# YiKwanwoo2/mycelium-fea-project

Hardware: AMD Instinct MI355X
Metric: DOF solved/sec + CG iters to 1e-8; SpMV achieved HBM GB/s vs roofline (higher is better)
Workload: dtype f64 (CG; f32 AMG V-cycle); 1 GPU; C3_1M: 6x8 tiles, 1062000 DOF, 1008054 free DOF, 364342 elements, load step 20/40; n_dof=1062000, n_free_dof=1008054, n_elems=364342, precond=gamg, parallelism=1gpu, cg_kernel=lanes, n_lanes=353600

## Files before the change

### mycelium-fea-project_amd/csrc/amg.hip

```cpp
#include "amg_dev.hpp"

namespace mfea {

__device__ __forceinline__ int64_t setup_block(int x1, int64_t nmain = -1) {
  if (!x1) return nmain < 0 ? xcd_block() : xcd_block_n(nmain);
  return (blockIdx.x & 7) ? -1 : (int64_t)(blockIdx.x >> 3);
}


template <int ND>
__device__ __forceinline__ double dinv_row(const AmgLevD& L, int64_t i) {
  const AmgMatD& A = L.A;
  double g = 0.0;
  if (i - (threadIdx.x & 63) < A.rg.hi) {
    int64_t base;
    int w;
    slice_of(A, i, base, w);
    if (i >= A.rg.lo && i < A.rg.hi) {
      double D[ND * ND], Di[ND * ND];
      bload<ND>(A.val32, A.npos, base, D);
      binv<ND>(D, Di);
#pragma unroll
      for (int c = 0; c < ND * ND; ++c) L.dinv32[i * (ND * ND) + c] = (float)Di[c];
      double rs[ND];
// ... 1265 lines not shown
      acc[2] = fma(r[a], r[a], acc[2]);
      acc[3] = fma(u[a], u[a], acc[3]);
    }
  }
  store_block_partial<BS>(acc, part_buf(part, FIRST ? 0 : ((j & 1) ^ 1)));
  if (FIRST && blockIdx.x == 0 && threadIdx.x == 0) {
    Slot s0;
    s0.v[0] = s0.v[1] = s0.v[2] = s0.v[3] = 0.0;
    s0.alpha = s0.beta = s0.res = 0.0;
    s0.flag = kInit;
    s0.pad = 0;
    slots[0] = s0;
  }
}

template <int ND, int BS>
__global__ __launch_bounds__(BS) void k_amg_rnorm(AmgCg cg, double* cpart) {
  double acc[4] = {0.0, 0.0, 0.0, 0.0};
  const int64_t stride = (int64_t)gridDim.x * BS;
  const int lane = threadIdx.x & 63;
  for (int64_t i = cg.lo64() + xcd_block() * BS + threadIdx.x; i - lane < cg.hi; i += stride) {
    if (i < cg.lo || i >= cg.hi) continue;
    double r[ND];
    vload<ND>(cg.r, i, r);
#pragma unroll
    for (int a = 0; a < ND; ++a) acc[2] = fma(r[a], r[a], acc[2]);
  }
  store_block_partial<BS>(acc, cpart);
}

template <int PU>
__global__ __launch_bounds__(64) void k_amg_gsum(const double* __restrict__ p, double* all, int rank, int zero_w,
                                                 double* gsend) {
  double S[4];
  wave_partials<PU>(p, S);
  const int lane = threadIdx.x;
  if (lane < zero_w && lane != rank) {
#pragma unroll
    for (int c = 0; c < 4; ++c) all[4 * lane + c] = 0.0;
// ... 4 lines not shown
      all[4 * rank + c] = S[c];
      gsend[c] = S[c];
    }
  }
}

template <int ND>
__global__ __launch_bounds__(kBlock) void k_amg_pack_u(AmgCg cg, AmgDist d) {
  const int64_t k = (int64_t)blockIdx.x * kBlock + threadIdx.x;
  if (k >= d.n_send) return;
  const int64_t i = d.send_rows[k];
#pragma unroll
  for (int a = 0; a < ND; ++a) d.usend[ND * k + a] = i >= 0 ? cg.u[ND * i + a] : 0.0;
}

template <int ND, int PU, int BS, bool DIST>
__global__ __launch_bounds__(BS) void k_amg_cg_update(int j, AmgLevD L0, AmgCg cg, Slot* slots,
                                                      SolveState* st, double* part, AmgDist d) {
  const int f0 = __builtin_nontemporal_load(&slots[j].flag);
  const double g0 = slots[j].v[0], a0 = slots[j].alpha;
  double tol2 = st->tol2;
  const int base_it = st->base, max_it = st->max_it, norm = st->norm;
  double S[4];
  if constexpr (DIST) {
    const int lane = threadIdx.x & 63;
    const double* g = d.gall[j & 1];
#pragma unroll
    for (int c = 0; c < 4; ++c) S[c] = wave_allsum(g[lane * 4 + c]);
  } else {
    wave_partials<PU>(part_buf(part, j & 1), S);
  }
  const int64_t stride = (int64_t)gridDim.x * BS;
  const int64_t i0 = cg.lo + (int64_t)blockIdx.x * BS + threadIdx.x;
  const bool x0_here = !cg.sweep && !L0.coarsest;
  const float om0 = x0_here ? (float)amg_omega_s(L0.omega) : 0.0f;
  double u[ND], w[ND], p[ND], s[ND], x[ND], r[ND];
  float Di[ND * ND];
  if (cg.hi > cg.lo) {
    const int64_t k = i0 < cg.hi ? i0 : cg.hi - 1;
    vload<ND>(cg.u, k, u);
    vload<ND>(cg.w, k, w);
    vload<ND>(cg.p, k, p);
    vload<ND>(cg.s, k, s);
    vload<ND>(cg.x, k, x);
    vload<ND>(cg.r, k, r);
    if (x0_here) dinv_load<ND>(L0.dinv32, k, Di);
  }
  if (norm == 1 && f0 == kInit) {
    tol2 = fmax(st->rtol2 * S[3], st->atol2);
    if (blockIdx.x == 0 && threadIdx.x == 0) {
      st->tol2 = tol2;
      st->res0 = S[3];
    }
  }
  const CgScalars cs = cg_scalars(S, f0, g0, a0, tol2, base_it + j, max_it, norm);
  cg_record(slots, j, S, cs);
  if (cs.status != kRun) return;
  const double alpha = cs.alpha, beta = cs.beta;
  for (int64_t i = i0; i < cg.hi; i += stride) {
    if (i != i0) {
      vload<ND>(cg.u, i, u);
      vload<ND>(cg.w, i, w);
      vload<ND>(cg.p, i, p);
      vload<ND>(cg.s, i, s);
      vload<ND>(cg.x, i, x);
      vload<ND>(cg.r, i, r);
      if (x0_here) dinv_load<ND>(L0.dinv32, i, Di);
    }
#pragma unroll
    for (int a = 0; a < ND; ++a) {
      p[a] = fma(beta, p[a], u[a]);
      s[a] = fma(beta, s[a], w[a]);
      x[a] = fma(alpha, p[a], x[a]);
      r[a] = fma(-alpha, s[a], r[a]);
    }
    vstore<ND>(cg.p, i, p);
    vstore<ND>(cg.s, i, s);
    vstore<ND>(cg.x, i, x);
    vstore<ND>(cg.r, i, r);
    if (x0_here) {
      float rf[ND], x0[ND];
#pragma unroll
      for (int a = 0; a < ND; ++a) rf[a] = (float)r[a];
      dinv_mul<ND>(Di, om0, rf, x0);
      vstore<ND>(L0.x, i, x0);
    } else {
      vcycle_entry<ND>(L0, cg, i, r);
    }
  }
}

template <int ND>
__global__ __launch_bounds__(kBlock) void k_amg_finish(AmgCg cg, double* __restrict__ x_row) {
// ... 444 lines not shown
    case 512: w_bs<ND, 512>(s, j, first, L0, cg, slots, part, d); break;
    case 576: w_bs<ND, 576>(s, j, first, L0, cg, slots, part, d); break;
    case 640: w_bs<ND, 640>(s, j, first, L0, cg, slots, part, d); break;
    case 704: w_bs<ND, 704>(s, j, first, L0, cg, slots, part, d); break;
    case 768: w_bs<ND, 768>(s, j, first, L0, cg, slots, part, d); break;
    case 1024: w_bs<ND, 1024>(s, j, first, L0, cg, slots, part, d); break;
    default: w_bs<ND, kCgBS>(s, j, first, L0, cg, slots, part, d); break;
  }
}
void launch_amg_cg_w(hipStream_t s, int nd, int j, bool first, const AmgLevD& L0, const AmgCg& cg,
                     Slot* slots, double* part, const AmgDist* d) {
  if (nd == 2) w_nd<2>(s, j, first, L0, cg, slots, part, d);
  else w_nd<3>(s, j, first, L0, cg, slots, part, d);
}

template <int ND>
static void rnorm_nd(hipStream_t s, const AmgCg& cg, double* cpart) {
  const dim3 g((unsigned)amg_w_grid(cg));
  switch (amg_w_block(cg)) {
    case 512: hipLaunchKernelGGL((k_amg_rnorm<ND, 512>), g, dim3(512), 0, s, cg, cpart); break;
    case 576: hipLaunchKernelGGL((k_amg_rnorm<ND, 576>), g, dim3(576), 0, s, cg, cpart); break;
    case 640: hipLaunchKernelGGL((k_amg_rnorm<ND, 640>), g, dim3(640), 0, s, cg, cpart); break;
    case 704: hipLaunchKernelGGL((k_amg_rnorm<ND, 704>), g, dim3(704), 0, s, cg, cpart); break;
    case 768: hipLaunchKernelGGL((k_amg_rnorm<ND, 768>), g, dim3(768), 0, s, cg, cpart); break;
    case 1024: hipLaunchKernelGGL((k_amg_rnorm<ND, 1024>), g, dim3(1024), 0, s, cg, cpart); break;
    default: hipLaunchKernelGGL((k_amg_rnorm<ND, kCgBS>), g, dim3(kCgBS), 0, s, cg, cpart); break;
  }
}
void launch_amg_rnorm(hipStream_t s, int nd, const AmgCg& cg, double* cpart) {
  if (nd == 2) rnorm_nd<2>(s, cg, cpart);
  else rnorm_nd<3>(s, cg, cpart);
}

void launch_amg_gsum(hipStream_t s, const AmgCg& cg, const double* part_q, const AmgDist& d, int q) {
  double* all = d.gall[q];
  const int r = d.rank, zw = d.zero_w;
  switch (pu_of_grid(amg_w_grid(cg))) {
    case 1: hipLaunchKernelGGL(k_amg_gsum<1>, dim3(1), dim3(64), 0, s, part_q, all, r, zw, d.gsend); break;
    case 2: hipLaunchKernelGGL(k_amg_gsum<2>, dim3(1), dim3(64), 0, s, part_q, all, r, zw, d.gsend); break;
    case 4: hipLaunchKernelGGL(k_amg_gsum<4>, dim3(1), dim3(64), 0, s, part_q, all, r, zw, d.gsend); break;
    default: hipLaunchKernelGGL(k_amg_gsum<8>, dim3(1), dim3(64), 0, s, part_q, all, r, zw, d.gsend); break;
  }
}

void launch_amg_pack_u(hipStream_t s, int nd, const AmgCg& cg, const AmgDist& d) {
  if (d.n_send <= 0) return;
  if (nd == 2) hipLaunchKernelGGL(k_amg_pack_u<2>, rows_grid(d.n_send), dim3(kBlock), 0, s, cg, d);
  else hipLaunchKernelGGL(k_amg_pack_u<3>, rows_grid(d.n_send), dim3(kBlock), 0, s, cg, d);
}

template <int ND, int BS, bool DIST>
static void upd_bs(hipStream_t s, int j, const AmgLevD& L0, const AmgCg& cg, Slot* slots,
                   SolveState* st, double* part, const AmgDist& d) {
  const int64_t gw = amg_w_grid(cg);
  int64_t gu = (cg.hi - cg.lo + BS - 1) / BS;
  gu = gu < 1 ? 1 : (gu > kCgMaxG ? kCgMaxG : gu);
  const dim3 g((unsigned)gu);
  switch (DIST ? 1 : pu_of_grid(gw)) {
    case 1: hipLaunchKernelGGL((k_amg_cg_update<ND, 1, BS, DIST>), g, dim3(BS), 0, s, j, L0, cg, slots, st, part, d); break;
    case 2: hipLaunchKernelGGL((k_amg_cg_update<ND, 2, BS, DIST>), g, dim3(BS), 0, s, j, L0, cg, slots, st, part, d); break;
    case 4: hipLaunchKernelGGL((k_amg_cg_update<ND, 4, BS, DIST>), g, dim3(BS), 0, s, j, L0, cg, slots, st, part, d); break;
    default: hipLaunchKernelGGL((k_amg_cg_update<ND, 8, BS, DIST>), g, dim3(BS), 0, s, j, L0, cg, slots, st, part, d); break;
  }
}
template <int ND>
static void upd_nd(hipStream_t s, int j, const AmgLevD& L0, const AmgCg& cg, Slot* slots,
                   SolveState* st, double* part, const AmgDist* d) {
  if (d) upd_bs<ND, kCgBS, true>(s, j, L0, cg, slots, st, part, *d);
  else upd_bs<ND, kCgBS, false>(s, j, L0, cg, slots, st, part, AmgDist{});
}
void launch_amg_cg_update(hipStream_t s, int nd, int j, const AmgLevD& L0, const AmgCg& cg, Slot* slots,
                          SolveState* st, double* part, const AmgDist* d) {
  if (nd == 2) upd_nd<2>(s, j, L0, cg, slots, st, part, d);
  else upd_nd<3>(s, j, L0, cg, slots, st, part, d);
}

void launch_amg_finish(hipStream_t s, int nd, const AmgCg& cg, double* x_row) {
  if (cg.hi <= cg.lo) return;
  if (nd == 2) hipLaunchKernelGGL(k_amg_finish<2>, rows_grid(cg.hi - cg.lo), dim3(kBlock), 0, s, cg, x_row);
  else hipLaunchKernelGGL(k_amg_finish<3>, rows_grid(cg.hi - cg.lo), dim3(kBlock), 0, s, cg, x_row);
}

template <class T>
__global__ __launch_bounds__(kBlock) void k_xpack(const T* __restrict__ src, const int32_t* __restrict__ idx,
                                                  int64_t n, int width, T* __restrict__ buf) {
  const int64_t k = (int64_t)blockIdx.x * kBlock + threadIdx.x;
  if (k >= n * width) return;
  const int64_t it = k / width, c = k - it * width;
  buf[k] = src[(int64_t)idx[it] * width + c];
// ... 92 lines not shown
```

### mycelium-fea-project_amd/csrc/amg_kernels.hpp

```cpp
#pragma once
#include <hip/hip_runtime.h>
#include <stdint.h>

#include "kernels.hpp"

namespace mfea {

struct RowRange {
  int64_t lo = 0, hi = 0;
  int64_t p0 = 0, p1 = 0;
  int64_t pf = 0, pl = 0;
  int64_t s0 = 0, s1 = 0;
  int64_t rows() const { return hi > lo ? hi - lo : 0; }
  __host__ __device__ int64_t lo64() const { return lo & ~(int64_t)63; }
  int64_t span() const { return hi > lo ? hi - lo64() : 0; }
  int64_t npos() const { return p1 > p0 ? p1 - p0 : 0; }
};

struct AmgMatD {
  int64_t n = 0;
  int64_t npos = 0;
  int32_t wmax = 0;
  RowRange rg;
  const int32_t* sptr = nullptr;
// ... 186 lines not shown
int amg_restrict_lanes(const AmgLevD& L);
int amg_op_lanes(const AmgLevD& L);
int amg_down_lanes(const AmgLevD& L);
int amg_up_lanes(const AmgLevD& L);
bool amg_compact_ok(const AmgLevD* lev, int nlev, int l0);
int amg_tail_level(const int64_t* rows, int nlev, int64_t max_rows);
void launch_amg_cg_init(hipStream_t s, int nd, const AmgLevD& L0, const AmgCg& cg, const double* b_row);
void launch_amg_cg_w(hipStream_t s, int nd, int j, bool first, const AmgLevD& L0, const AmgCg& cg,
                     Slot* slots, double* part, const AmgDist* d = nullptr);
void launch_amg_row0_inverse(hipStream_t s, const AmgCg& cg, int32_t* inv, int64_t n_rows);
void launch_amg_start(hipStream_t s, int nd, const SellOp& op, const uint8_t* code, double dy_top, double dy_bot,
                      const CgVecs& v, double* partials, unsigned* ticket, double* red_out, const AmgLevD& L0,
                      const AmgCg& cg, const int32_t* inv, double rtol, double atol, int norm, int max_it,
                      double reg, SolveState* st, double* zero, int64_t nzero);
void launch_amg_rnorm(hipStream_t s, int nd, const AmgCg& cg, double* cpart);
void launch_amg_gsum(hipStream_t s, const AmgCg& cg, const double* part_q, const AmgDist& d, int q);
void launch_amg_pack_u(hipStream_t s, int nd, const AmgCg& cg, const AmgDist& d);
void launch_amg_cg_update(hipStream_t s, int nd, int j, const AmgLevD& L0, const AmgCg& cg,
                          Slot* slots, SolveState* st, double* part,
                          const AmgDist* d = nullptr);
void launch_amg_finish(hipStream_t s, int nd, const AmgCg& cg, double* x_row);
int64_t amg_w_grid(const AmgCg& cg);

}
```

### mycelium-fea-project_amd/csrc/capi.hip

```cpp
#include <hip/hip_runtime.h>
#include <rccl/rccl.h>

#include <algorithm>
#include <deque>
#include <chrono>
#include <cmath>
#include <cstdio>
#include <cstring>
#include <memory>
#include <string>
#include <thread>
#include <vector>

#include "amg.hpp"
#include "amg_kernels.hpp"
#include "kernels.hpp"
#include "mfea_debug.h"
#include "mfea.h"
#include "partition.hpp"
#include "records.hpp"
#include "run.hpp"
#include "symbolic.hpp"

using namespace mfea;
// ... 128 lines not shown
  double amg_build_s = 0.0;
  double amg_excess_s = 0.0;
  bool amg_stale = false;
  bool amg_reused = false;
  int64_t amg_seen_gen = -1;
  DevBuf<int32_t> amg_i;
  DevBuf<double> amg_d;
  DevBuf<float> amg_f;
  std::vector<AmgLevD> amg_lev;
  DevBuf<AmgLevD> amg_levd;
  bool amg_om_own = false;
  bool amg_om_spatial = false;
  int amg_tail = 0;
  int amg_first = 1;
  AmgCg amg_cg;
  int amg_kind = MFEA_PC_GAMG;
  SweepPlan sweep;
  SweepD swd;
  DevBuf<int32_t> sw_i;
  DevBuf<float> sw_f;
  DevBuf<double> sw_y;
  const int32_t* amg_a0_ptr = nullptr;
  const int32_t* amg_a0_a = nullptr;
  AmgHalo amg_halo;
  AmgDist amg_dist;
  DevBuf<int32_t> amg_hi;
  DevBuf<double> amg_hd;
  AmgRank amg_rank;
  PosList g_a0;
  std::vector<int32_t> g_row0;
// ... 67 lines not shown
  int64_t op_gen = 0;
  struct {
    bool ok = false;
    int64_t act_gen = -1;
    Material mat{};
    int asm_kernel = -1;
  } k_from;
  int last_precond = -1;
  int64_t op_kept_steps = 0;
  int64_t amg_setup_kept = 0;
  int opt_amg_close = 1;
  int64_t amg_close_hits = 0;
  int amg_last_cycles = 0;
  int opt_amg_start = 1;
  int64_t amg_start_fused = 0;
  bool setup_skipped = false;
  Material graph_batch_mat{};
  bool asm_pending = false;
  DevBuf<double> d_dy;
  bool spec_on = false;
  bool spec_used = false;
  bool spec_launched = false;
  double spec_strain = 0.0;
  bool ev_on = false;
  double ev_strain = 0.0, ev_tie = 0.0, ev_lam_max = 0.0;
  int32_t ev_index = 0;
  int opt_event_scratch = 1;
  hipEvent_t poll[2] = {};
  int64_t n_active = 0;
  bool act_all = false;
// ... 1131 lines not shown
    const int64_t nf = nlev ? pl.lev[0].A.n : 0;
    pt.amg_cg.n = nf;
    pt.amg_cg.lo = rk && nlev ? rk->lo[0] : 0;
    pt.amg_cg.hi = rk && nlev ? rk->hi[0] : nf;
    pt.amg_cg.w_block = h->opt_amg_w_block;
    pt.amg_cg.w_k = amg_w_k(pl);
    pt.amg_cg.cycle = h->opt_amg_cycle;
    pt.amg_cg.coll = pt.amg_coll.kc;
    pt.amg_cg.row0 = I(row0 ? *row0 : pl.row0);
    pt.amg_cg.x = D((size_t)nd * nf);
    pt.amg_cg.p = D((size_t)nd * nf);
    pt.amg_cg.s = D((size_t)nd * nf);
    pt.amg_cg.w = D((size_t)nd * nf);
    pt.amg_cg.r = D((size_t)nd * nf);
    pt.amg_cg.u = F((size_t)nd * nf);
    pt.amg_mg = AmgMergeD{};
    if (pt.amg_mplan.on) {
      const AmgMerge& M = pt.amg_mplan;
      AmgMergeD& g = pt.amg_mg;
      g.n1 = M.n1;
      g.n2 = M.n2;
      g.DQ = mat(M.DQ, false, true);
      g.DQ.rg = row_range(M.DQ, 0, M.DQ.n);
      g.U = mat(M.U, false, true);
      g.U.rg = row_range(M.U, 0, M.U.n);
      g.dq_dst = I(M.dq_dst);
      g.dq_split = M.dq_split;
      g.dq_ext = I(M.dq_ext);
      g.dq_ptr = I(M.dq_l.ptr);
      g.dq_a = I(M.dq_l.a);
// ... 136 lines not shown
  w.up_pos = put(sp.up_pos);
  float* fp = pt.sw_f.ptr;
  w.pv = fp;
  w.dt = fp + (size_t)ne * nb2;
  w.lov = w.dt + (size_t)ne * ns;
  w.upv = w.lov + nlo * nb2;
  HIPC(hipMemsetAsync(fp, 0, pt.sw_f.n * sizeof(float), s));
  w.y = pt.sw_y.ptr;
  HIPC(hipMemsetAsync(w.y, 0, pt.sw_y.n * sizeof(double), s));
  pt.amg_cg.sweep = 1;
  HIPC(hipGetLastError());
  HIPC(hipStreamSynchronize(s));
  return 0;
}

void launch_precond(mfea_handle* h, Part& pt, const int32_t* gate) {
  if (pt.amg_cg.sweep) launch_sweep(h->stream, pt.amg.nd, pt.swd, pt.amg_cg, gate);
  else launch_amg_vcycle(h->stream, pt.amg.nd, pt.amg_lev.data(), (int)pt.amg_lev.size(), pt.amg_cg, pt.amg_tail, gate,
                         0, pt.amg_mg.on ? &pt.amg_mg : nullptr);
}

int upload_sweep(mfea_handle* h, Part& pt, int kind);

static bool active_subset(const std::vector<uint8_t>& a, const std::vector<uint8_t>& b) {
  if (a.size() != b.size()) return false;
  for (size_t e = 0; e < a.size(); ++e)
    if (a[e] && !b[e]) return false;
  return true;
}

std::string build_sweep_bounded(const AmgPlan& plan, int piece_len, SweepPlan& sp) {
  for (int m = piece_len;; m = std::max(1, m / 2)) {
    const std::string err = build_sweep(plan, m, sp);
    if (!err.empty() || sp.colors <= kSweepMaxColors) return err;
    if (m == 1) return "sweep plan: more than 32 colours";
// ... 70 lines not shown
  pt.amg_reused = false;
  if (!dm && pt.amg_lev.size() > 1) RC(enqueue_fmask(h, pt));
  clk.lap("floating mask");
  if (!dm) pt.amg_seen_gen = h->act_gen;
  pt.amg_sub_gen = dm ? -1 : h->act_sub_gen;
  pt.amg_key_count = (int64_t)std::count(key.begin(), key.end(), (uint8_t)1);
  ++pt.amg_gen;
  *rebuilt = true;
  return 0;
}

void enqueue_amg_iteration(mfea_handle* h, Part& pt, int j, bool profile) {
  hipStream_t s = h->stream;
  const int nd = pt.amg.nd;
  const AmgLevD& L0 = pt.amg_lev[0];
  launch_amg_cg_update(s, nd, j, L0, pt.amg_cg, pt.slots.ptr, pt.state.ptr, pt.cg_part.ptr);
  (void)profile;
  launch_precond(h, pt, nullptr);
  launch_amg_cg_w(s, nd, j, profile, L0, pt.amg_cg, pt.slots.ptr, pt.cg_part.ptr);
}

int xchg_u(mfea_handle* h) {
  hipStream_t s = h->stream;
  const int64_t nd = part0(h).amg.nd;
  if (h->world > 1) {
    Part& pt = part0(h);
    const PartPlan& pl = pt.plan;
    if (pl.xpeers.empty()) return 0;
    NCCLC(ncclGroupStart());
    for (size_t i = 0; i < pl.xpeers.size(); ++i) {
      if (pl.xsend_cnt[i])
        NCCLC(ncclSend(pt.amg_dist.usend + nd * pl.xsend_off[i], (size_t)(nd * pl.xsend_cnt[i]), ncclFloat64,
                       pl.xpeers[i], h->comm, s));
      if (pl.xrecv_cnt[i])
// ... 70 lines not shown
  HIPC(hipGetLastError());
  return xchg_sums(h, q);
}

int enqueue_amg_dist_chunk(mfea_handle* h, int chunk) {
  for (int j = 0; j < chunk; ++j) RC(enqueue_amg_dist_iteration(h, j));
  for (auto& pp : h->parts) launch_cg_advance(h->stream, chunk, pp->slots.ptr, pp->state.ptr, pp->mirror);
  HIPC(hipGetLastError());
  return 0;
}

void enqueue_amg_chunk(mfea_handle* h, Part& pt, int chunk, bool close) {
  hipStream_t s = h->stream;
  const int nd = pt.amg.nd;
  const AmgLevD& L0 = pt.amg_lev[0];
  for (int j = 0; j < chunk; ++j) {
    launch_precond(h, pt, nullptr);
    launch_amg_cg_w(s, nd, j, false, L0, pt.amg_cg, pt.slots.ptr, pt.cg_part.ptr);
    launch_amg_cg_update(s, nd, j + 1, L0, pt.amg_cg, pt.slots.ptr, pt.state.ptr, pt.cg_part.ptr);
  }
  if (close) launch_amg_rnorm(s, nd, pt.amg_cg, cg_part_buf(pt, 2));
  launch_cg_advance(s, chunk, pt.slots.ptr, pt.state.ptr, pt.mirror, 1, close ? cg_part_buf(pt, 2) : nullptr,
                    close ? (int)amg_w_grid(pt.amg_cg) : 0);
}

void enqueue_amg_setup(mfea_handle* h, Part& pt, double reg) {
  hipStream_t s = h->stream;
  const int nd = pt.amg.nd, nlev = (int)pt.amg_lev.size();
  const bool compact = pt.amg_cg.cycle == 1 && nlev > 1 && pt.amg_lev[0].compact;
  const bool fused = compact && h->opt_amg_fuse_setup && !pt.amg_cg.sweep;
  launch_amg_a0(s, nd, pt.amg_lev[0], sell_op(pt), pt.amg_cg.row0, pt.amg_a0_ptr, pt.amg_a0_a, reg,
                fused && pt.amg_lev[0].a0full);
  if (pt.amg_cg.sweep) {
    launch_sweep_setup(s, nd, pt.swd, pt.amg_lev[0]);
    return;
  }
// ... 8 lines not shown
  if (pt.amg_mg.on && !merged_done) launch_amg_merge_setup(s, nd, pt.amg_lev.data(), pt.amg_mg);
}

uint64_t fnv1a(uint64_t k, const void* p, size_t n) {
  const unsigned char* b = static_cast<const unsigned char*>(p);
  size_t i = 0;
  for (; i + 8 <= n; i += 8) {
    uint64_t w;
    std::memcpy(&w, b + i, 8);
    k = (k ^ w) * 1099511628211ULL;
  }
  for (; i < n; ++i) k = (k ^ b[i]) * 1099511628211ULL;
  return k;
}

void launch_precond(mfea_handle* h, Part& pt, const int32_t* gate);
int enqueue_post_work(mfea_handle* h, double max_strain);

void enqueue_amg_entry(mfea_handle* h, Part& pt, bool skip_init = false) {
  hipStream_t s = h->stream;
  const int nd = pt.amg.nd;
  const AmgLevD& L0 = pt.amg_lev[0];
  if (!skip_init) launch_amg_cg_init(s, nd, L0, pt.amg_cg, cg_vecs(pt).r[0]);
  launch_precond(h, pt, nullptr);
  launch_amg_cg_w(s, nd, 0, true, L0, pt.amg_cg, pt.slots.ptr, pt.cg_part.ptr);
  launch_amg_cg_update(s, nd, 0, L0, pt.amg_cg, pt.slots.ptr, pt.state.ptr, pt.cg_part.ptr);
}

void enqueue_step_head(mfea_handle* h, Part& pt, const mfea_solve_opts* o) {
  hipStream_t s = h->stream;
  const Pattern& P = pt.P;
  (void)hipMemcpyAsync(h->d_dy.ptr, h->h_red + 14, 2 * sizeof(double), hipMemcpyHostToDevice, s);
  AsmRhs q{};
  q.code = pt.code.ptr;
  q.top_end = P.n_free + P.n_top;
  q.bot_end = P.n_nodes - P.n_ghost;
  q.dyp = h->d_dy.ptr;
  q.nf = P.n_free;
  q.r = pt.r.ptr;
  q.x = pt.x.ptr;
  q.partials = pt.partials.ptr;
// ... 24 lines not shown
                           const mfea_solve_opts* head = nullptr, const mfea_solve_opts* start = nullptr,
                           int tail = -1, int tag = 0, bool close = false, bool skip_init = false) {
  hipStream_t s = h->stream;
  uint64_t k = k0;
  const int form = keep ? 1 : 0;
  k = fnv1a(k, &form, sizeof form);
  if (keep && !entry && !head && !start && tail < 0) return 0;
  if (entry) {
    const CgVecs v = cg_vecs(pt);
    const void* eptrs[4] = {v.r[0], pt.slots.ptr, pt.state.ptr, pt.cg_part.ptr};
    k = fnv1a(k, eptrs, sizeof eptrs);
    k = fnv1a(k, &pt.amg_cg, sizeof pt.amg_cg);
    k = fnv1a(k, &pt.amg_kind, sizeof pt.amg_kind);
    const int si = skip_init ? 1 : 0;
    k = fnv1a(k, &si, sizeof si);
  }
  if (start) {
    const double sd[3] = {start->rtol, start->atol, start->reg};
    const int si[2] = {start->norm, start->max_it};
    const void* sp[3] = {pt.red.ptr, pt.state.ptr, pt.cg_part.ptr};
    k = fnv1a(k ^ 0x5a5a, sd, sizeof sd);
    k = fnv1a(k, si, sizeof si);
    k = fnv1a(k, sp, sizeof sp);
  }
  if (head) {
    const void* hptrs[10] = {pt.xyz_d.ptr, pt.s_elem.ptr, pt.active.ptr, pt.code.ptr, pt.r.ptr,
                             pt.x.ptr, pt.partials.ptr, pt.red.ptr, h->d_dy.ptr, h->h_red};
    k = fnv1a(k, hptrs, sizeof hptrs);
    const double hd[3] = {head->rtol, head->atol, head->reg};
    const int hi[2] = {head->norm, head->max_it};
// ... 116 lines not shown
      launch_amg_start(s, nd, op, pt.code.ptr, dy_top, dy_bot, v, pt.partials.ptr, tix(pt, 0), pt.red.ptr,
                       pt.amg_lev[0], pt.amg_cg, pt.amg_inv.ptr, o->rtol, o->atol, o->norm, o->max_it, o->reg,
                       pt.state.ptr, pt.cg_part.ptr, 2 * 4 * kCgMaxPartials);
      ++h->amg_start_fused;
    } else {
      if (!rhs_done)
        launch_cg_rhs(s, op, pt.code.ptr, dy_top, dy_bot, o->reg, 2, v, pt.partials.ptr, tix(pt, 0), pt.red.ptr);
      if (!start_in_graph)
        launch_cg_init_finalize(s, pt.red.ptr, o->rtol, o->atol, o->norm, o->max_it, o->reg, pt.state.ptr,
                                pt.cg_part.ptr, 2 * 4 * kCgMaxPartials);
    }
  }
  RC(phase_event(h, h->ev[2], s));
  const bool entry = h->opt_graph && h->opt_setup_entry && !h->opt_phase_times;
  const bool close = h->opt_amg_close && o->norm == MFEA_NORM_UNPRECONDITIONED && pt.amg_kind == MFEA_PC_GAMG;
  const int tag = -1000 - (int)(pt.amg_gen % 1000000) - (close ? 4000000 : 0);
  const int planned = std::min(o->max_it, pt.amg_last_iters > 0 ? pt.amg_last_iters : 16);
  const int need = close ? std::max(0, planned - 1) : std::max(1, planned);
  int cycles = 1;
  const bool batch = h->spec_on && !h->ev_on && !h->spec_used && h->opt_batch_graph && !h->opt_phase_times &&
                     o->chunk <= 0 && need < mfea_handle::kRemGraphs && h->opt_graph;
  const bool combo = batch && entry && h->opt_combo_graph;
  if (combo) h->h_state[0].done = 0;
  if (h->opt_graph) {
    const bool split = combo && !keep && h->opt_keep_operator && !head;
    if (split) RC(launch_amg_setup_graph(h, pt, o->reg, skey, false));
    RC(launch_amg_setup_graph(h, pt, o->reg, skey, keep || split, entry, head ? o : nullptr,
                              start_in_graph && !fused_start ? o : nullptr, combo ? need : -1, tag, close,
                              fused_start));
  } else if (!keep) {
    enqueue_amg_setup(h, pt, o->reg);
// ... 7 lines not shown
  HIPC(hipGetLastError());
  const bool no_graph = !h->opt_graph;
  SolveState fin;
  int rc;
  const auto drive_t0 = std::chrono::steady_clock::now();
  auto finish = [&]() -> int {
    launch_amg_finish(s, nd, pt.amg_cg, pt.x.ptr);
    HIPC(hipGetLastError());
    return spec_post(h);
  };
  if (no_graph) {
    rc = drive_planned(h, chunk, o->max_it, need - 1,
                       [&]() -> int {
                         enqueue_amg_chunk(h, pt, chunk, close);
                         cycles += chunk;
                         HIPC(hipGetLastError());
                         return 0;
                       },
                       &fin, finish);
  } else {
    auto capture = [&](hipGraphExec_t* ge, int n) -> int {
      hipGraph_t g;
      HIPC(hipStreamBeginCapture(s, hipStreamCaptureModeThreadLocal));
      enqueue_amg_chunk(h, pt, n, close);
      HIPC(hipStreamEndCapture(s, &g));
      hipError_t e = hipGraphInstantiate(ge, g, nullptr, nullptr, 0);
      (void)hipGraphDestroy(g);
      HIPC(e);
      return 0;
    };
// ... 38 lines not shown
        HIPC(hipStreamBeginCapture(s, hipStreamCaptureModeThreadLocal));
        enqueue_amg_chunk(h, pt, need, close);
        launch_amg_finish(s, nd, pt.amg_cg, pt.x.ptr);
        const int prc = enqueue_post_work(h, h->spec_strain);
        const hipError_t ec = hipStreamEndCapture(s, &g);
        RC(prc);
        HIPC(ec);
        hipError_t e = hipGraphInstantiate(&h->graph_batch[need], g, nullptr, nullptr, 0);
        (void)hipGraphDestroy(g);
        HIPC(e);
      }
      rc = drive_batch(h, chunk, o->max_it, need,
                       [&]() -> int {
                         if (!combo) HIPC(hipGraphLaunch(h->graph_batch[need], s));
                         cycles += need;
                         return 0;
                       },
                       [&](int n) -> int {
                         HIPC(hipGraphLaunch(h->graph, s));
                         cycles += n;
                         return 0;
                       },
                       &fin, finish, combo);
    } else {
      const int odd = need == 0 ? 0 : rem;
      if ((exact_rem || need == 0) && h->graph_rem[odd] == nullptr) RC(capture(&h->graph_rem[odd], odd));
      rc = drive_sized(h, big, chunk, o->max_it, need - 1,
                       [&](int n) -> int {
                         HIPC(hipGraphLaunch(n == chunk ? h->graph : n == big ? h->graph_big : h->graph_rem[n], s));
                         cycles += n;
                         return 0;
                       },
                       &fin, finish, exact_rem, close);
    }
  }
  if (rc) return rc;
  h->amg_last_cycles = cycles;
  if (fin.status == 0 && fin.closed) ++h->amg_close_hits;
  if (fin.status != 0) RC(spec_undo(h));
  clk.lap("solve (setup + iterations)", fin.iters);
  if (fin.status != 0 && pt.amg_reused) {
    pt.amg_stale = true;
    RC(sync_stream(h));
    return solve_amg(h, dy_top, dy_bot, o, st);
  }
  if (pt.amg_lev.size() > 1 && pt.amg_kind == MFEA_PC_GAMG &&
      omega_suspect(h, fin.status, o->max_it, std::max(pt.amg_build_iters, pt.amg_last_iters)))
    return omega_retry(h, [&]() { return solve_amg(h, dy_top, dy_bot, o, st); });
  if (fin.status == 0) pt.amg_last_iters = fin.iters;
  if (fin.status == 0 && !pt.amg_reused) {
// ... 2198 lines not shown
    h->opt_part_slack = value / 100.0;
    rebuild = true;
  }
  else if (n == "keep_operator") {
    if (value != 0 && value != 1) return fail(MFEA_EINVAL, "keep_operator: 0 or 1");
    h->opt_keep_operator = (int)value;
  }
  else if (n == "amg_close") {
    if (value != 0 && value != 1) return fail(MFEA_EINVAL, "amg_close: 0 or 1");
    h->opt_amg_close = (int)value;
  }
  else if (n == "amg_start") {
    if (value != 0 && value != 1) return fail(MFEA_EINVAL, "amg_start: 0 or 1");
    h->opt_amg_start = (int)value;
  }
  else return fail(MFEA_EINVAL, "unknown option " + n);
  if (n != "phase_times" && n != "run_register" && !(n == "keep_operator" && value == 1) &&
      n != "amg_close" && n != "amg_start")
    drop_kept(h);
  destroy_graph(h);
  if (rebuild) {
    if (!h->dirty && h->Ecount) {
      RC(set_device(h));
      RC(gather_active(h, h->active_host));
    }
    h->dirty = true;
  }
  return 0;
}

int mfea_debug_amg_vcycle(mfea_handle* h, const double* r, double* u) {
  if (!h || !r || !u) return fail(MFEA_EINVAL, "NULL argument");
  RC(set_device(h));
// ... 178 lines not shown
    *value = h->opt_amg_dist >= 0 ? h->opt_amg_dist : h->amg_auto.choice;
  else if (n == "amg_rep_rows") *value = h->opt_amg_rep_rows;
  else if (n == "cc_tile") *value = h->opt_cc_tile;
  else if (n == "asm_kernel") *value = h->opt_asm_kernel;
  else if (n == "spec_post") *value = h->opt_spec_post;
  else if (n == "setup_entry") *value = h->opt_setup_entry;
  else if (n == "batch_graph") *value = h->opt_batch_graph;
  else if (n == "step_graph") *value = h->opt_step_graph;
  else if (n == "graph_start") *value = h->opt_graph_start;
  else if (n == "combo_graph") *value = h->opt_combo_graph;
  else if (n == "keep_operator") *value = h->opt_keep_operator;
  else if (n == "op_kept_steps") *value = h->op_kept_steps;
  else if (n == "amg_setup_kept") *value = h->amg_setup_kept;
  else if (n == "amg_close") *value = h->opt_amg_close;
  else if (n == "amg_start") *value = h->opt_amg_start;
  else if (n == "amg_start_fused") *value = h->amg_start_fused;
  else if (n == "amg_close_hits") *value = h->amg_close_hits;
  else if (n == "amg_last_cycles") *value = h->amg_last_cycles;
  else if (n == "asm_colours") {
    *value = 0;
    for (auto& pp : h->parts) *value = std::max<int64_t>(*value, pp->ec_state > 0 ? pp->ec.colors : 0);
  }
  else if (n == "amg_dist_cycle") *value = h->opt_amg_dist_cycle;
  else if (n == "dist_sums") *value = h->opt_dist_sums;
  else if (n == "part_slack_pct") *value = (int64_t)std::llround(h->opt_part_slack * 100.0);
  else return fail(MFEA_EINVAL, "unknown option " + n);
  return 0;
}

int mfea_debug_global_active(mfea_handle* h, uint8_t* out) {
// ... 198 lines not shown
```

### mycelium-fea-project_amd/csrc/cg.hip

```cpp
#include "device_util.hpp"
#include "kernels.hpp"

namespace mfea {

static_assert(kCgMaxG == 512, "launch_cg_iter dispatches PU up to 8");

int cg_block_size(int64_t) { return kCgBS; }
int64_t cg_grid(int64_t rows) {
  int64_t g = (rows + kCgBS - 1) / kCgBS;
  return g < 1 ? 1 : (g > kCgMaxG ? kCgMaxG : g);
}

template <bool BLOCK>
__device__ __forceinline__ void apply_minv(const double* __restrict__ dinv, int64_t row,
                                           const double r[3], double u[3]) {
  if (BLOCK) {
    double B[6];
#pragma unroll
    for (int c = 0; c < 6; ++c) B[c] = dinv[6 * row + c];
    sym_apply(B, r, u);
  } else {
#pragma unroll
    for (int a = 0; a < 3; ++a) u[a] = dinv[3 * row + a] * r[a];
  }
// ... 344 lines not shown
    *host = *st;
    return;
  }
  if (cpart && st->norm == 0 && cg_close_converged(rr, st->tol2)) {
    st->iters = st->base + chunk + shift;
    st->res_final = rr;
    st->status = 0;
    st->done = 1;
    st->closed = 1;
    slots[0].flag = kStop;
    slots[shift].flag = kStop;
    *host = *st;
    return;
  }
  slots[shift] = slots[chunk + shift];
  st->base += chunk;
}

void launch_cg_rhs(hipStream_t s, const SellOp& op, const uint8_t* code, double dy_top,
                   double dy_bot, double reg, int precond, const CgVecs& v, double* partials,
                   unsigned* ticket, double* red_out) {
  const dim3 grid((unsigned)grid_rows(op.N > 0 ? op.N : 1));
  if (precond == 2)
    hipLaunchKernelGGL(k_amg_rhs, grid, dim3(kBlock), 0, s, op, code, dy_top, dy_bot, v, partials, ticket,
                       red_out);
  else if (precond == 1)
    hipLaunchKernelGGL(k_cg_rhs<true>, grid, dim3(kBlock), 0, s, op, code, dy_top, dy_bot, reg, v,
                       partials, ticket, red_out);
  else
    hipLaunchKernelGGL(k_cg_rhs<false>, grid, dim3(kBlock), 0, s, op, code, dy_top, dy_bot, reg, v,
// ... 54 lines not shown
```

Baseline: 985.4 million DOF/s.

## Defer CG p/x updates by storing preconditioned residuals and replaying in batches

```diff
diff --git a/mycelium-fea-project_amd/csrc/amg.hip b/mycelium-fea-project_amd/csrc/amg.hip
--- a/mycelium-fea-project_amd/csrc/amg.hip
+++ b/mycelium-fea-project_amd/csrc/amg.hip
@@ -1303,8 +1303,67 @@
   }
 }
 
-template <int ND, int BS>
-__global__ __launch_bounds__(BS) void k_amg_rnorm(AmgCg cg, double* cpart) {
+struct PxLive {
+  double alpha[kAmgPxSlots], beta[kAmgPxSlots];
+  int64_t off[kAmgPxSlots];
+  int n;
+};
+__device__ __forceinline__ void px_records(const Slot* __restrict__ slots, const AmgPx& px, PxLive& L) {
+  if (threadIdx.x < 64) {
+    const int t = threadIdx.x, k = px.k0 + t;
+    bool run = false;
+    double a = 0.0, b = 0.0;
+    if (t < px.cnt) {
+      const Slot& rec = slots[k + 1];
+      run = rec.flag == kRun && rec.pad == 0;
+      a = rec.alpha;
+      b = rec.beta;
+    }
+    const unsigned long long m = __ballot(run);
+    if (run) {
+      const int q = __popcll(m & ((1ull << t) - 1ull));
+      L.alpha[q] = a;
+      L.beta[q] = b;
+      L.off[q] = (int64_t)amg_px_slot(k) * px.stride;
+    }
+    if (t == 0) L.n = __popcll(m);
+  }
+  __syncthreads();
+}
+template <int ND>
+__device__ __forceinline__ void px_row(const AmgCg& cg, const AmgPx& px, const PxLive& L, int64_t i) {
+  const int n = L.n;
+  if (n == 0) return;
+  double p[ND], x[ND];
+  vload<ND>(cg.p, i, p);
+  vload<ND>(cg.x, i, x);
+#pragma unroll 4
+  for (int t = 0; t < n; ++t) {
+    double u[ND];
+    vload<ND>(px.uh + L.off[t], i, u);
+    const double alpha = L.alpha[t], beta = L.beta[t];
+#pragma unroll
+    for (int a = 0; a < ND; ++a) {
+      p[a] = fma(beta, p[a], u[a]);
+      x[a] = fma(alpha, p[a], x[a]);
+    }
+  }
+  vstore<ND>(cg.p, i, p);
+  vstore<ND>(cg.x, i, x);
+}
+template <int ND>
+__global__ __launch_bounds__(kCgBS) void k_amg_px_replay(AmgCg cg, const Slot* slots, AmgPx px) {
+  __shared__ PxLive live;
+  px_records(slots, px, live);
+  const int64_t stride = (int64_t)gridDim.x * kCgBS;
+  for (int64_t i = cg.lo + (int64_t)blockIdx.x * kCgBS + threadIdx.x; i < cg.hi; i += stride)
+    px_row<ND>(cg, px, live, i);
+}
+
+template <int ND, int BS, bool REPLAY = false>
+__global__ __launch_bounds__(BS) void k_amg_rnorm(AmgCg cg, double* cpart, const Slot* slots, AmgPx px) {
+  __shared__ PxLive live;
+  if constexpr (REPLAY) px_records(slots, px, live);
   double acc[4] = {0.0, 0.0, 0.0, 0.0};
   const int64_t stride = (int64_t)gridDim.x * BS;
   const int lane = threadIdx.x & 63;
@@ -1312,6 +1371,7 @@
     if (i < cg.lo || i >= cg.hi) continue;
     double r[ND];
     vload<ND>(cg.r, i, r);
+    if constexpr (REPLAY) px_row<ND>(cg, px, live, i);
 #pragma unroll
     for (int a = 0; a < ND; ++a) acc[2] = fma(r[a], r[a], acc[2]);
   }
@@ -1346,7 +1406,7 @@
   for (int a = 0; a < ND; ++a) d.usend[ND * k + a] = i >= 0 ? cg.u[ND * i + a] : 0.0;
 }
 
-template <int ND, int PU, int BS, bool DIST>
+template <int ND, int PU, int BS, bool DIST, bool LAZY = false>
 __global__ __launch_bounds__(BS) void k_amg_cg_update(int j, AmgLevD L0, AmgCg cg, Slot* slots,
                                                       SolveState* st, double* part, AmgDist d) {
   const int f0 = __builtin_nontemporal_load(&slots[j].flag);
@@ -1370,11 +1430,11 @@
   float Di[ND * ND];
   if (cg.hi > cg.lo) {
     const int64_t k = i0 < cg.hi ? i0 : cg.hi - 1;
-    vload<ND>(cg.u, k, u);
+    if constexpr (!LAZY) vload<ND>(cg.u, k, u);
     vload<ND>(cg.w, k, w);
-    vload<ND>(cg.p, k, p);
+    if constexpr (!LAZY) vload<ND>(cg.p, k, p);
     vload<ND>(cg.s, k, s);
-    vload<ND>(cg.x, k, x);
+    if constexpr (!LAZY) vload<ND>(cg.x, k, x);
     vload<ND>(cg.r, k, r);
     if (x0_here) dinv_load<ND>(L0.dinv32, k, Di);
   }
@@ -1391,24 +1451,24 @@
   const double alpha = cs.alpha, beta = cs.beta;
   for (int64_t i = i0; i < cg.hi; i += stride) {
     if (i != i0) {
-      vload<ND>(cg.u, i, u);
+      if constexpr (!LAZY) vload<ND>(cg.u, i, u);
       vload<ND>(cg.w, i, w);
-      vload<ND>(cg.p, i, p);
+      if constexpr (!LAZY) vload<ND>(cg.p, i, p);
       vload<ND>(cg.s, i, s);
-      vload<ND>(cg.x, i, x);
+      if constexpr (!LAZY) vload<ND>(cg.x, i, x);
       vload<ND>(cg.r, i, r);
       if (x0_here) dinv_load<ND>(L0.dinv32, i, Di);
     }
 #pragma unroll
     for (int a = 0; a < ND; ++a) {
-      p[a] = fma(beta, p[a], u[a]);
+      if constexpr (!LAZY) p[a] = fma(beta, p[a], u[a]);
       s[a] = fma(beta, s[a], w[a]);
-      x[a] = fma(alpha, p[a], x[a]);
+      if constexpr (!LAZY) x[a] = fma(alpha, p[a], x[a]);
       r[a] = fma(-alpha, s[a], r[a]);
     }
-    vstore<ND>(cg.p, i, p);
+    if constexpr (!LAZY) vstore<ND>(cg.p, i, p);
     vstore<ND>(cg.s, i, s);
-    vstore<ND>(cg.x, i, x);
+    if constexpr (!LAZY) vstore<ND>(cg.x, i, x);
     vstore<ND>(cg.r, i, r);
     if (x0_here) {
       float rf[ND], x0[ND];
@@ -1883,22 +1943,34 @@
   else w_nd<3>(s, j, first, L0, cg, slots, part, d);
 }
 
-template <int ND>
-static void rnorm_nd(hipStream_t s, const AmgCg& cg, double* cpart) {
+template <int ND, bool REPLAY>
+static void rnorm_nd(hipStream_t s, const AmgCg& cg, double* cpart, const Slot* slots, const AmgPx& px) {
   const dim3 g((unsigned)amg_w_grid(cg));
   switch (amg_w_block(cg)) {
-    case 512: hipLaunchKernelGGL((k_amg_rnorm<ND, 512>), g, dim3(512), 0, s, cg, cpart); break;
-    case 576: hipLaunchKernelGGL((k_amg_rnorm<ND, 576>), g, dim3(576), 0, s, cg, cpart); break;
-    case 640: hipLaunchKernelGGL((k_amg_rnorm<ND, 640>), g, dim3(640), 0, s, cg, cpart); break;
-    case 704: hipLaunchKernelGGL((k_amg_rnorm<ND, 704>), g, dim3(704), 0, s, cg, cpart); break;
-    case 768: hipLaunchKernelGGL((k_amg_rnorm<ND, 768>), g, dim3(768), 0, s, cg, cpart); break;
-    case 1024: hipLaunchKernelGGL((k_amg_rnorm<ND, 1024>), g, dim3(1024), 0, s, cg, cpart); break;
-    default: hipLaunchKernelGGL((k_amg_rnorm<ND, kCgBS>), g, dim3(kCgBS), 0, s, cg, cpart); break;
+    case 512: hipLaunchKernelGGL((k_amg_rnorm<ND, 512, REPLAY>), g, dim3(512), 0, s, cg, cpart, slots, px); break;
+    case 576: hipLaunchKernelGGL((k_amg_rnorm<ND, 576, REPLAY>), g, dim3(576), 0, s, cg, cpart, slots, px); break;
+    case 640: hipLaunchKernelGGL((k_amg_rnorm<ND, 640, REPLAY>), g, dim3(640), 0, s, cg, cpart, slots, px); break;
+    case 704: hipLaunchKernelGGL((k_amg_rnorm<ND, 704, REPLAY>), g, dim3(704), 0, s, cg, cpart, slots, px); break;
+    case 768: hipLaunchKernelGGL((k_amg_rnorm<ND, 768, REPLAY>), g, dim3(768), 0, s, cg, cpart, slots, px); break;
+    case 1024: hipLaunchKernelGGL((k_amg_rnorm<ND, 1024, REPLAY>), g, dim3(1024), 0, s, cg, cpart, slots, px); break;
+    default: hipLaunchKernelGGL((k_amg_rnorm<ND, kCgBS, REPLAY>), g, dim3(kCgBS), 0, s, cg, cpart, slots, px); break;
   }
 }
 void launch_amg_rnorm(hipStream_t s, int nd, const AmgCg& cg, double* cpart) {
-  if (nd == 2) rnorm_nd<2>(s, cg, cpart);
-  else rnorm_nd<3>(s, cg, cpart);
+  if (nd == 2) rnorm_nd<2, false>(s, cg, cpart, nullptr, AmgPx{});
+  else rnorm_nd<3, false>(s, cg, cpart, nullptr, AmgPx{});
+}
+void launch_amg_rnorm_px(hipStream_t s, int nd, const AmgCg& cg, double* cpart, const Slot* slots,
+                         const AmgPx& px) {
+  if (nd == 2) rnorm_nd<2, true>(s, cg, cpart, slots, px);
+  else rnorm_nd<3, true>(s, cg, cpart, slots, px);
+}
+void launch_amg_px_replay(hipStream_t s, int nd, const AmgCg& cg, const Slot* slots, const AmgPx& px) {
+  if (cg.hi <= cg.lo) return;
+  int64_t g = (cg.hi - cg.lo + kCgBS - 1) / kCgBS;
+  g = g > kCgMaxG ? kCgMaxG : g;
+  if (nd == 2) hipLaunchKernelGGL(k_amg_px_replay<2>, dim3((unsigned)g), dim3(kCgBS), 0, s, cg, slots, px);
+  else hipLaunchKernelGGL(k_amg_px_replay<3>, dim3((unsigned)g), dim3(kCgBS), 0, s, cg, slots, px);
 }
 
 void launch_amg_gsum(hipStream_t s, const AmgCg& cg, const double* part_q, const AmgDist& d, int q) {
@@ -1918,7 +1990,7 @@
   else hipLaunchKernelGGL(k_amg_pack_u<3>, rows_grid(d.n_send), dim3(kBlock), 0, s, cg, d);
 }
 
-template <int ND, int BS, bool DIST>
+template <int ND, int BS, bool DIST, bool LAZY = false>
 static void upd_bs(hipStream_t s, int j, const AmgLevD& L0, const AmgCg& cg, Slot* slots,
                    SolveState* st, double* part, const AmgDist& d) {
   const int64_t gw = amg_w_grid(cg);
@@ -1926,22 +1998,24 @@
   gu = gu < 1 ? 1 : (gu > kCgMaxG ? kCgMaxG : gu);
   const dim3 g((unsigned)gu);
   switch (DIST ? 1 : pu_of_grid(gw)) {
-    case 1: hipLaunchKernelGGL((k_amg_cg_update<ND, 1, BS, DIST>), g, dim3(BS), 0, s, j, L0, cg, slots, st, part, d); break;
-    case 2: hipLaunchKernelGGL((k_amg_cg_update<ND, 2, BS, DIST>), g, dim3(BS), 0, s, j, L0, cg, slots, st, part, d); break;
-    case 4: hipLaunchKernelGGL((k_amg_cg_update<ND, 4, BS, DIST>), g, dim3(BS), 0, s, j, L0, cg, slots, st, part, d); break;
-    default: hipLaunchKernelGGL((k_amg_cg_update<ND, 8, BS, DIST>), g, dim3(BS), 0, s, j, L0, cg, slots, st, part, d); break;
+    case 1: hipLaunchKernelGGL((k_amg_cg_update<ND, 1, BS, DIST, LAZY>), g, dim3(BS), 0, s, j, L0, cg, slots, st, part, d); break;
+    case 2: hipLaunchKernelGGL((k_amg_cg_update<ND, 2, BS, DIST, LAZY>), g, dim3(BS), 0, s, j, L0, cg, slots, st, part, d); break;
+    case 4: hipLaunchKernelGGL((k_amg_cg_update<ND, 4, BS, DIST, LAZY>), g, dim3(BS), 0, s, j, L0, cg, slots, st, part, d); break;
+    default: hipLaunchKernelGGL((k_amg_cg_update<ND, 8, BS, DIST, LAZY>), g, dim3(BS), 0, s, j, L0, cg, slots, st, part, d); break;
   }
 }
 template <int ND>
 static void upd_nd(hipStream_t s, int j, const AmgLevD& L0, const AmgCg& cg, Slot* slots,
-                   SolveState* st, double* part, const AmgDist* d) {
+                   SolveState* st, double* part, const AmgDist* d, bool lazy) {
   if (d) upd_bs<ND, kCgBS, true>(s, j, L0, cg, slots, st, part, *d);
+  else if (lazy) upd_bs<ND, kCgBS, false, true>(s, j, L0, cg, slots, st, part, AmgDist{});
   else upd_bs<ND, kCgBS, false>(s, j, L0, cg, slots, st, part, AmgDist{});
 }
 void launch_amg_cg_update(hipStream_t s, int nd, int j, const AmgLevD& L0, const AmgCg& cg, Slot* slots,
-                          SolveState* st, double* part, const AmgDist* d) {
-  if (nd == 2) upd_nd<2>(s, j, L0, cg, slots, st, part, d);
-  else upd_nd<3>(s, j, L0, cg, slots, st, part, d);
+                          SolveState* st, double* part, const AmgDist* d, bool lazy) {
+  lazy = lazy && !d && !cg.sweep && !L0.coarsest;
+  if (nd == 2) upd_nd<2>(s, j, L0, cg, slots, st, part, d, lazy);
+  else upd_nd<3>(s, j, L0, cg, slots, st, part, d, lazy);
 }
 
 void launch_amg_finish(hipStream_t s, int nd, const AmgCg& cg, double* x_row) {
diff --git a/mycelium-fea-project_amd/csrc/amg_kernels.hpp b/mycelium-fea-project_amd/csrc/amg_kernels.hpp
--- a/mycelium-fea-project_amd/csrc/amg_kernels.hpp
+++ b/mycelium-fea-project_amd/csrc/amg_kernels.hpp
@@ -224,11 +224,22 @@
                       const AmgCg& cg, const int32_t* inv, double rtol, double atol, int norm, int max_it,
                       double reg, SolveState* st, double* zero, int64_t nzero);
 void launch_amg_rnorm(hipStream_t s, int nd, const AmgCg& cg, double* cpart);
+constexpr int kAmgPxSlots = 17;
+struct AmgPx {
+  const float* uh = nullptr;
+  int64_t stride = 0;
+  int k0 = 0;
+  int cnt = 0;
+};
+__host__ __device__ inline int amg_px_slot(int k) { return k == 0 ? 0 : 1 + (k - 1) % (kAmgPxSlots - 1); }
+void launch_amg_rnorm_px(hipStream_t s, int nd, const AmgCg& cg, double* cpart, const Slot* slots,
+                         const AmgPx& px);
+void launch_amg_px_replay(hipStream_t s, int nd, const AmgCg& cg, const Slot* slots, const AmgPx& px);
 void launch_amg_gsum(hipStream_t s, const AmgCg& cg, const double* part_q, const AmgDist& d, int q);
 void launch_amg_pack_u(hipStream_t s, int nd, const AmgCg& cg, const AmgDist& d);
 void launch_amg_cg_update(hipStream_t s, int nd, int j, const AmgLevD& L0, const AmgCg& cg,
                           Slot* slots, SolveState* st, double* part,
-                          const AmgDist* d = nullptr);
+                          const AmgDist* d = nullptr, bool lazy = false);
 void launch_amg_finish(hipStream_t s, int nd, const AmgCg& cg, double* x_row);
 int64_t amg_w_grid(const AmgCg& cg);
 
diff --git a/mycelium-fea-project_amd/csrc/capi.hip b/mycelium-fea-project_amd/csrc/capi.hip
--- a/mycelium-fea-project_amd/csrc/capi.hip
+++ b/mycelium-fea-project_amd/csrc/capi.hip
@@ -166,6 +166,8 @@
   int amg_tail = 0;
   int amg_first = 1;
   AmgCg amg_cg;
+  float* amg_uh = nullptr;
+  int64_t amg_uh_stride = 0;
   int amg_kind = MFEA_PC_GAMG;
   SweepPlan sweep;
   SweepD swd;
@@ -263,6 +265,8 @@
   int amg_last_cycles = 0;
   int opt_amg_start = 1;
   int64_t amg_start_fused = 0;
+  int opt_amg_lazy_px = 1;
+  int64_t amg_px_replays = 0;
   bool setup_skipped = false;
   Material graph_batch_mat{};
   bool asm_pending = false;
@@ -1424,6 +1428,8 @@
     pt.amg_cg.w = D((size_t)nd * nf);
     pt.amg_cg.r = D((size_t)nd * nf);
     pt.amg_cg.u = F((size_t)nd * nf);
+    pt.amg_uh_stride = (int64_t)amg_al((size_t)nd * nf);
+    pt.amg_uh = !rk && nlev > 1 ? F((size_t)kAmgPxSlots * pt.amg_uh_stride) : nullptr;
     pt.amg_mg = AmgMergeD{};
     if (pt.amg_mplan.on) {
       const AmgMerge& M = pt.amg_mplan;
@@ -1590,11 +1596,30 @@
   return 0;
 }
 
-void launch_precond(mfea_handle* h, Part& pt, const int32_t* gate) {
-  if (pt.amg_cg.sweep) launch_sweep(h->stream, pt.amg.nd, pt.swd, pt.amg_cg, gate);
-  else launch_amg_vcycle(h->stream, pt.amg.nd, pt.amg_lev.data(), (int)pt.amg_lev.size(), pt.amg_cg, pt.amg_tail, gate,
+void launch_precond(mfea_handle* h, Part& pt, const int32_t* gate, const AmgCg* cg) {
+  const AmgCg& c = cg ? *cg : pt.amg_cg;
+  if (pt.amg_cg.sweep) launch_sweep(h->stream, pt.amg.nd, pt.swd, c, gate);
+  else launch_amg_vcycle(h->stream, pt.amg.nd, pt.amg_lev.data(), (int)pt.amg_lev.size(), c, pt.amg_tail, gate,
                          0, pt.amg_mg.on ? &pt.amg_mg : nullptr);
 }
+
+bool amg_lazy(const mfea_handle* h, const Part& pt) {
+  return h->opt_amg_lazy_px && pt.amg_uh && !pt.amg_cg.sweep && !pt.amg_lev.empty() && !pt.amg_lev[0].coarsest;
+}
+AmgCg px_cg(const Part& pt, int k) {
+  AmgCg c = pt.amg_cg;
+  c.u = pt.amg_uh + (int64_t)amg_px_slot(k) * pt.amg_uh_stride;
+  return c;
+}
+AmgPx px_of(const Part& pt, int k0, int cnt) {
+  AmgPx px;
+  px.uh = pt.amg_uh;
+  px.stride = pt.amg_uh_stride;
+  px.k0 = k0;
+  px.cnt = cnt;
+  return px;
+}
+int px_replays(int chunk) { return 1 + (chunk > 0 ? (chunk - 1) / (kAmgPxSlots - 1) : 0); }
 
 int upload_sweep(mfea_handle* h, Part& pt, int kind);
 
@@ -1695,10 +1720,12 @@
   hipStream_t s = h->stream;
   const int nd = pt.amg.nd;
   const AmgLevD& L0 = pt.amg_lev[0];
-  launch_amg_cg_update(s, nd, j, L0, pt.amg_cg, pt.slots.ptr, pt.state.ptr, pt.cg_part.ptr);
+  const bool lazy = amg_lazy(h, pt);
+  const AmgCg cg = lazy ? px_cg(pt, j) : pt.amg_cg;
+  launch_amg_cg_update(s, nd, j, L0, cg, pt.slots.ptr, pt.state.ptr, pt.cg_part.ptr, nullptr, lazy);
   (void)profile;
-  launch_precond(h, pt, nullptr);
-  launch_amg_cg_w(s, nd, j, profile, L0, pt.amg_cg, pt.slots.ptr, pt.cg_part.ptr);
+  launch_precond(h, pt, nullptr, &cg);
+  launch_amg_cg_w(s, nd, j, profile, L0, cg, pt.slots.ptr, pt.cg_part.ptr);
 }
 
 int xchg_u(mfea_handle* h) {
@@ -1799,12 +1826,21 @@
   hipStream_t s = h->stream;
   const int nd = pt.amg.nd;
   const AmgLevD& L0 = pt.amg_lev[0];
+  const bool lazy = amg_lazy(h, pt);
+  int k0 = 0;
   for (int j = 0; j < chunk; ++j) {
-    launch_precond(h, pt, nullptr);
-    launch_amg_cg_w(s, nd, j, false, L0, pt.amg_cg, pt.slots.ptr, pt.cg_part.ptr);
-    launch_amg_cg_update(s, nd, j + 1, L0, pt.amg_cg, pt.slots.ptr, pt.state.ptr, pt.cg_part.ptr);
-  }
-  if (close) launch_amg_rnorm(s, nd, pt.amg_cg, cg_part_buf(pt, 2));
+    const AmgCg cg = lazy ? px_cg(pt, j + 1) : pt.amg_cg;
+    launch_precond(h, pt, nullptr, &cg);
+    launch_amg_cg_w(s, nd, j, false, L0, cg, pt.slots.ptr, pt.cg_part.ptr);
+    launch_amg_cg_update(s, nd, j + 1, L0, cg, pt.slots.ptr, pt.state.ptr, pt.cg_part.ptr, nullptr, lazy);
+    if (lazy && (j + 1) % (kAmgPxSlots - 1) == 0 && j + 1 < chunk) {
+      launch_amg_px_replay(s, nd, pt.amg_cg, pt.slots.ptr, px_of(pt, k0, j + 2 - k0));
+      k0 = j + 2;
+    }
+  }
+  if (lazy && close) launch_amg_rnorm_px(s, nd, pt.amg_cg, cg_part_buf(pt, 2), pt.slots.ptr, px_of(pt, k0, chunk + 1 - k0));
+  else if (lazy) launch_amg_px_replay(s, nd, pt.amg_cg, pt.slots.ptr, px_of(pt, k0, chunk + 1 - k0));
+  else if (close) launch_amg_rnorm(s, nd, pt.amg_cg, cg_part_buf(pt, 2));
   launch_cg_advance(s, chunk, pt.slots.ptr, pt.state.ptr, pt.mirror, 1, close ? cg_part_buf(pt, 2) : nullptr,
                     close ? (int)amg_w_grid(pt.amg_cg) : 0);
 }
@@ -1843,7 +1879,6 @@
   return k;
 }
 
-void launch_precond(mfea_handle* h, Part& pt, const int32_t* gate);
 int enqueue_post_work(mfea_handle* h, double max_strain);
 
 void enqueue_amg_entry(mfea_handle* h, Part& pt, bool skip_init = false) {
@@ -1851,9 +1886,11 @@
   const int nd = pt.amg.nd;
   const AmgLevD& L0 = pt.amg_lev[0];
   if (!skip_init) launch_amg_cg_init(s, nd, L0, pt.amg_cg, cg_vecs(pt).r[0]);
-  launch_precond(h, pt, nullptr);
-  launch_amg_cg_w(s, nd, 0, true, L0, pt.amg_cg, pt.slots.ptr, pt.cg_part.ptr);
-  launch_amg_cg_update(s, nd, 0, L0, pt.amg_cg, pt.slots.ptr, pt.state.ptr, pt.cg_part.ptr);
+  const bool lazy = amg_lazy(h, pt);
+  const AmgCg cg = lazy ? px_cg(pt, 0) : pt.amg_cg;
+  launch_precond(h, pt, nullptr, &cg);
+  launch_amg_cg_w(s, nd, 0, true, L0, cg, pt.slots.ptr, pt.cg_part.ptr);
+  launch_amg_cg_update(s, nd, 0, L0, cg, pt.slots.ptr, pt.state.ptr, pt.cg_part.ptr, nullptr, lazy);
 }
 
 void enqueue_step_head(mfea_handle* h, Part& pt, const mfea_solve_opts* o) {
@@ -1908,6 +1945,9 @@
     k = fnv1a(k, &pt.amg_kind, sizeof pt.amg_kind);
     const int si = skip_init ? 1 : 0;
     k = fnv1a(k, &si, sizeof si);
+    const int lz = amg_lazy(h, pt) ? 1 : 0;
+    k = fnv1a(k, &lz, sizeof lz);
+    k = fnv1a(k, &pt.amg_uh, sizeof pt.amg_uh);
   }
   if (start) {
     const double sd[3] = {start->rtol, start->atol, start->reg};
@@ -2054,7 +2094,9 @@
   RC(phase_event(h, h->ev[2], s));
   const bool entry = h->opt_graph && h->opt_setup_entry && !h->opt_phase_times;
   const bool close = h->opt_amg_close && o->norm == MFEA_NORM_UNPRECONDITIONED && pt.amg_kind == MFEA_PC_GAMG;
-  const int tag = -1000 - (int)(pt.amg_gen % 1000000) - (close ? 4000000 : 0);
+  const bool lazy = amg_lazy(h, pt);
+  const int tag = -1000 - (int)(pt.amg_gen % 1000000) - (close ? 4000000 : 0) - (lazy ? 8000000 : 0);
+  int64_t replays = 0;
   const int planned = std::min(o->max_it, pt.amg_last_iters > 0 ? pt.amg_last_iters : 16);
   const int need = close ? std::max(0, planned - 1) : std::max(1, planned);
   int cycles = 1;
@@ -2092,6 +2134,7 @@
                        [&]() -> int {
                          enqueue_amg_chunk(h, pt, chunk, close);
                          cycles += chunk;
+                         if (lazy) replays += px_replays(chunk);
                          HIPC(hipGetLastError());
                          return 0;
                        },
@@ -2160,11 +2203,13 @@
                        [&]() -> int {
                          if (!combo) HIPC(hipGraphLaunch(h->graph_batch[need], s));
                          cycles += need;
+                         if (lazy) replays += px_replays(need);
                          return 0;
                        },
                        [&](int n) -> int {
                          HIPC(hipGraphLaunch(h->graph, s));
                          cycles += n;
+                         if (lazy) replays += px_replays(chunk);
                          return 0;
                        },
                        &fin, finish, combo);
@@ -2175,11 +2220,13 @@
                        [&](int n) -> int {
                          HIPC(hipGraphLaunch(n == chunk ? h->graph : n == big ? h->graph_big : h->graph_rem[n], s));
                          cycles += n;
+                         if (lazy) replays += px_replays(n);
                          return 0;
                        },
                        &fin, finish, exact_rem, close);
     }
   }
+  h->amg_px_replays += replays;
   if (rc) return rc;
   h->amg_last_cycles = cycles;
   if (fin.status == 0 && fin.closed) ++h->amg_close_hits;
@@ -4408,9 +4455,17 @@
     if (value != 0 && value != 1) return fail(MFEA_EINVAL, "amg_start: 0 or 1");
     h->opt_amg_start = (int)value;
   }
+  else if (n == "amg_lazy_px") {
+    if (value != 0 && value != 1) return fail(MFEA_EINVAL, "amg_lazy_px: 0 or 1");
+    h->opt_amg_lazy_px = (int)value;
+  }
+  else if (n == "amg_big_chunk") {
+    if (value < 2 || value >= mfea_handle::kRemGraphs) return fail(MFEA_EINVAL, "amg_big_chunk: 2..63");
+    h->opt_amg_big_chunk = (int)value;
+  }
   else return fail(MFEA_EINVAL, "unknown option " + n);
   if (n != "phase_times" && n != "run_register" && !(n == "keep_operator" && value == 1) &&
-      n != "amg_close" && n != "amg_start")
+      n != "amg_close" && n != "amg_start" && n != "amg_lazy_px" && n != "amg_big_chunk")
     drop_kept(h);
   destroy_graph(h);
   if (rebuild) {
@@ -4619,6 +4674,10 @@
   else if (n == "amg_setup_kept") *value = h->amg_setup_kept;
   else if (n == "amg_close") *value = h->opt_amg_close;
   else if (n == "amg_start") *value = h->opt_amg_start;
+  else if (n == "amg_lazy_px") *value = h->opt_amg_lazy_px;
+  else if (n == "amg_big_chunk") *value = h->opt_amg_big_chunk;
+  else if (n == "amg_px_replays") *value = h->amg_px_replays;
+  else if (n == "amg_px_slots") *value = kAmgPxSlots;
   else if (n == "amg_start_fused") *value = h->amg_start_fused;
   else if (n == "amg_close_hits") *value = h->amg_close_hits;
   else if (n == "amg_last_cycles") *value = h->amg_last_cycles;
diff --git a/mycelium-fea-project_amd/csrc/cg.hip b/mycelium-fea-project_amd/csrc/cg.hip
--- a/mycelium-fea-project_amd/csrc/cg.hip
+++ b/mycelium-fea-project_amd/csrc/cg.hip
@@ -382,6 +382,7 @@
     return;
   }
   slots[shift] = slots[chunk + shift];
+  slots[shift].pad = 1;
   st->base += chunk;
 }
 
```

Measured after the change: 1.021 billion DOF/s (median of 6 runs). +3.6%, better.
